# MarvinLvn/CPC2

Measured on AMD Instinct MI355X. Metric: audio-seconds/sec CPC training (1.28 s @16 kHz, 128 neg), higher is better.
Workload: dtype f32

## Files before the change

cpc2_amd/csrc/gru.hip:

```cpp
#include "common.h"
#include "coop.h"
#include "recurrent.h"

#include <algorithm>
#include <cstdlib>

namespace cpc {

__global__ void gru_pack_fwd_kernel(const float *w, float4 *wf, int H)
{
    const int total = 3 * H * (H / 4);
    for (int idx = blockIdx.x * blockDim.x + threadIdx.x; idx < total; idx += gridDim.x * blockDim.x) {
        const int j = idx % H;
        const int g = (idx / H) % 3;
        const int k4 = idx / (3 * H);
        const float *src = w + (long)(g * H + j) * H + 4 * k4;
        wf[idx] = make_float4(src[0], src[1], src[2], src[3]);
    }
}

__global__ void gru_pack_bwd_kernel(const float *w, float4 *wb, int H)
{
    const int total = (3 * H / 4) * H;
    for (int idx = blockIdx.x * blockDim.x + threadIdx.x; idx < total; idx += gridDim.x * blockDim.x) {
        const int j = idx % H;
        const int g4 = idx / H;
        wb[idx] = make_float4(w[(long)(4 * g4) * H + j], w[(long)(4 * g4 + 1) * H + j], w[(long)(4 * g4 + 2) * H + j],
                              w[(long)(4 * g4 + 3) * H + j]);
    }
}

__device__ __forceinline__ float sigmoidf_(float x) { return 1.f / (1.f + expf(-x)); }

struct GruArgs {
    const float *gi;
    const float4 *wpack;
    const float *whh;
    const float *bhh;
    const float *h0;
    float *out;
    float *hall;
    float *gates;
    float *hn;
    float *hlast;
    int N, T, H;
    int hp, kq;
    const float *dout;
    float *dgi;
    float *dgh;
};

__global__ void gru_fwd_kernel(GruArgs a)
{
    extern __shared__ __attribute__((aligned(16))) float smem[];
    const int H = a.H, T = a.T, hp = a.hp, kq = a.kq;
    float *hs = smem;
    float *red = smem + ((H + 3) / 4) * 4;
    const int j = threadIdx.x % hp, q = threadIdx.x / hp;
    const bool act = j < H;
    const int n = blockIdx.x;
    const int k4_per = (H / 4 + kq - 1) / kq;
    const int k4_lo = q * k4_per, k4_hi = min(H / 4, k4_lo + k4_per);

    float hprev = 0.f;
    float bh[3] = {0.f, 0.f, 0.f};
    if (act && q == 0) {
        hprev = a.h0 != nullptr ? a.h0[(long)n * H + j] : 0.f;
        hs[j] = hprev;
        a.hall[((long)n * (T + 1)) * H + j] = hprev;
        bh[0] = a.bhh[j]; bh[1] = a.bhh[H + j]; bh[2] = a.bhh[2 * H + j];
    }
    __syncthreads();

    for (int t = 0; t < T; ++t) {
        float acc0 = 0.f, acc1 = 0.f, acc2 = 0.f;
        if (act) {
            const float4 *wp = a.wpack + j;
#pragma unroll 4
            for (int k4 = k4_lo; k4 < k4_hi; ++k4) {
                const float4 wr = wp[(long)(k4 * 3 + 0) * H];
                const float4 wz = wp[(long)(k4 * 3 + 1) * H];
                const float4 wn = wp[(long)(k4 * 3 + 2) * H];
                const float4 h4 = reinterpret_cast<const float4 *>(hs)[k4];
                acc0 = fmaf(wr.x, h4.x, fmaf(wr.y, h4.y, fmaf(wr.z, h4.z, fmaf(wr.w, h4.w, acc0))));
                acc1 = fmaf(wz.x, h4.x, fmaf(wz.y, h4.y, fmaf(wz.z, h4.z, fmaf(wz.w, h4.w, acc1))));
                acc2 = fmaf(wn.x, h4.x, fmaf(wn.y, h4.y, fmaf(wn.z, h4.z, fmaf(wn.w, h4.w, acc2))));
            }
            red[(q * 3 + 0) * hp + j] = acc0;
            red[(q * 3 + 1) * hp + j] = acc1;
            red[(q * 3 + 2) * hp + j] = acc2;
        }
        __syncthreads();
        if (act && q == 0) {
            float g0 = bh[0], g1 = bh[1], g2 = bh[2];
            for (int qq = 0; qq < kq; ++qq) {
                g0 += red[(qq * 3 + 0) * hp + j];
                g1 += red[(qq * 3 + 1) * hp + j];
                g2 += red[(qq * 3 + 2) * hp + j];
            }
            const long row = (long)n * T + t;
            const float *g = a.gi + row * 3 * H;
            const float r = sigmoidf_(g[j] + g0);
            const float z = sigmoidf_(g[H + j] + g1);
            const float c = tanhf(g[2 * H + j] + r * g2);
            const float hv = (1.f - z) * c + z * hprev;
            float *gs = a.gates + row * 3 * H;
            gs[j] = r; gs[H + j] = z; gs[2 * H + j] = c;
            a.hn[row * H + j] = g2;
            a.out[row * H + j] = hv;
            a.hall[((long)n * (T + 1) + t + 1) * H + j] = hv;
            hs[j] = hv;
            hprev = hv;
        }
        __syncthreads();
    }
    if (act && q == 0 && a.hlast != nullptr) a.hlast[(long)n * H + j] = hprev;
}

__global__ void gru_bwd_kernel(GruArgs a)
{
    extern __shared__ __attribute__((aligned(16))) float smem[];
    const int H = a.H, T = a.T, hp = a.hp, kq = a.kq;
    float *dg = smem;
    float *red = smem + 3 * H;
    const int j = threadIdx.x % hp, q = threadIdx.x / hp;
    const bool act = j < H;
    const int n = blockIdx.x;
    const int g4_total = 3 * H / 4;
    const int g4_per = (g4_total + kq - 1) / kq;
    const int g4_lo = q * g4_per, g4_hi = min(g4_total, g4_lo + g4_per);

    float carry = 0.f;
    if (act && q == 0) {
        float *zr = a.dgh + ((long)n * (T + 1) + T) * 3 * H;
        zr[j] = 0.f; zr[H + j] = 0.f; zr[2 * H + j] = 0.f;
    }
    for (int t = T - 1; t >= 0; --t) {
        float keep = 0.f;
        if (act && q == 0) {
            const long row = (long)n * T + t;
            const float dh = a.dout[row * H + j] + carry;
            const float *gs = a.gates + row * 3 * H;
            const float r = gs[j], z = gs[H + j], c = gs[2 * H + j];
            const float hnv = a.hn[row * H + j];
            const float hp_ = a.hall[((long)n * (T + 1) + t) * H + j];
            const float dc = dh * (1.f - z);
            const float dz = dh * (hp_ - c);
            const float dpn = dc * (1.f - c * c);
            const float dpr = dpn * hnv * r * (1.f - r);
            const float dpz = dz * z * (1.f - z);
            const float dhn = dpn * r;
            keep = dh * z;
            float *gi = a.dgi + row * 3 * H;
            gi[j] = dpr; gi[H + j] = dpz; gi[2 * H + j] = dpn;
            float *gh = a.dgh + ((long)n * (T + 1) + t) * 3 * H;
            gh[j] = dpr; gh[H + j] = dpz; gh[2 * H + j] = dhn;
            dg[j] = dpr; dg[H + j] = dpz; dg[2 * H + j] = dhn;
        }
        __syncthreads();
        if (act) {
            float acc = 0.f;
            const float4 *wp = a.wpack + j;
#pragma unroll 4
            for (int g4 = g4_lo; g4 < g4_hi; ++g4) {
                const float4 w4 = wp[(long)g4 * H];
                const float4 d4 = reinterpret_cast<const float4 *>(dg)[g4];
                acc = fmaf(w4.x, d4.x, fmaf(w4.y, d4.y, fmaf(w4.z, d4.z, fmaf(w4.w, d4.w, acc))));
            }
            red[q * hp + j] = acc;
        }
        __syncthreads();
        if (act && q == 0) {
            float sum = keep;
            for (int qq = 0; qq < kq; ++qq) sum += red[qq * hp + j];
            carry = sum;
        }
    }
}

struct GruCoopArgs {
    GruArgs g;
    gu64_t *comm;
    unsigned epoch0;
    int groups, xcd_map;
    int *err;
    int fault;
};

template <int H, int NB> __global__ __launch_bounds__(512) void gru_fwd_coop_kernel(GruCoopArgs ca)
{
    using C = CoopCfg<H>;
    constexpr int QS = C::QS, U = C::U, G = C::G;
    constexpr int KP = NB * H / 512 > 0 ? NB * H / 512 : 1;
    static_assert(NB <= QS, "one finishing lane per window");
    __shared__ __attribute__((aligned(16))) float hs[2][NB][C::LDH];
    const GruArgs &a = ca.g;
    const int T = a.T;
    int group, member;
    coop_who<G>(ca.groups, ca.xcd_map, group, member);
    const int tid = threadIdx.x;
    const int q = tid & (QS - 1), u = tid / QS;
    const int j = member * U + u;
    const int n0 = group * NB;

    f32x2 w[3][16];
#pragma unroll
    for (int g = 0; g < 3; ++g)
#pragma unroll
        for (int i4 = 0; i4 < 8; ++i4) {
            const float4 v = *reinterpret_cast<const float4 *>(a.whh + (long)(g * H + j) * H + q * 32 + 4 * i4);
            w[g][2 * i4] = pk_lo(v); w[g][2 * i4 + 1] = pk_hi(v);
        }
    const float bh0 = a.bhh[j], bh1 = a.bhh[H + j], bh2 = a.bhh[2 * H + j];

    for (int idx = tid; idx < NB * H; idx += 512) {
        const int s = idx / H, k = idx - s * H;
        const int n = n0 + s;
        const float v = (n < a.N && a.h0 != nullptr) ? a.h0[(long)n * H + k] : 0.f;
        hs[0][s][coop_pad(k)] = v;
        if (n < a.N && (k / U) == member) a.hall[((long)n * (T + 1)) * H + k] = v;
    }
    __syncthreads();

    const int ns = n0 + q;
    const bool mine = q < NB && ns < a.N;
    float gin0 = 0.f, gin1 = 0.f, gin2 = 0.f;
    if (mine) {
        const float *gp = a.gi + (long)ns * T * 3 * H;
        gin0 = gp[j]; gin1 = gp[H + j]; gin2 = gp[2 * H + j];
    }
    bool dead = false;
    for (int t = 0; t < T; ++t) {
        const int cur = t & 1, nxt = cur ^ 1;
        const float gi0 = gin0, gi1 = gin1, gi2 = gin2;
        if (mine && t + 1 < T) {
            const float *gp = a.gi + ((long)ns * T + t + 1) * 3 * H;
            gin0 = gp[j]; gin1 = gp[H + j]; gin2 = gp[2 * H + j];
        }
        float acc[NB][3];
#pragma unroll
        for (int s = 0; s < NB; ++s) {
            f32x2 a2[3] = {f32x2{0.f, 0.f}, f32x2{0.f, 0.f}, f32x2{0.f, 0.f}};
#pragma unroll
            for (int i4 = 0; i4 < 8; ++i4) {
                const float4 h4 = *reinterpret_cast<const float4 *>(&hs[cur][s][q * 36 + 4 * i4]);
#pragma unroll
                for (int g = 0; g < 3; ++g)
                    a2[g] = pk_fma(w[g][2 * i4 + 1], pk_hi(h4), pk_fma(w[g][2 * i4], pk_lo(h4), a2[g]));
            }
#pragma unroll
            for (int g = 0; g < 3; ++g) acc[s][g] = coop_group_sum<QS>(a2[g].x + a2[g].y);
        }
        if (q < NB) {
            float g0 = 0.f, g1 = 0.f, g2 = 0.f;
#pragma unroll
            for (int s = 0; s < NB; ++s)
                if (s == q) { g0 = acc[s][0]; g1 = acc[s][1]; g2 = acc[s][2]; }
            g0 += bh0; g1 += bh1; g2 += bh2;
            const float hp = hs[cur][q][coop_pad(j)];
            const float r = sigmoidf_(gi0 + g0);
            const float z = sigmoidf_(gi1 + g1);
            const float c = tanhf(gi2 + r * g2);
            float hv = (1.f - z) * c + z * hp;
            if (dead) hv = NAN;
            COOP_GLOBAL gu64_t *slot = (COOP_GLOBAL gu64_t *)(ca.comm + coop_fwd_slot<H, NB>(group, nxt, member, u, q));
            if (!(ca.fault && group == 0 && member == 0 && t == 1))
                __hip_atomic_store(slot, ((gu64_t)(ca.epoch0 + (unsigned)(t + 1)) << 32) | (gu64_t)__float_as_uint(mine ? hv : 0.f),
                                   __ATOMIC_RELAXED, __HIP_MEMORY_SCOPE_AGENT);
            if (mine) {
                const long row = (long)ns * T + t;
                float *gs = a.gates + row * 3 * H;
                gs[j] = r; gs[H + j] = z; gs[2 * H + j] = c;
                a.hn[row * H + j] = g2;
                a.out[row * H + j] = hv;
                a.hall[((long)ns * (T + 1) + t + 1) * H + j] = hv;
            }
        }
        if (t + 1 < T) {
            COOP_GLOBAL gu64_t *slot[KP];
#pragma unroll
            for (int i = 0; i < KP; ++i) {
                const int idx = tid + 512 * i;
                slot[i] = (COOP_GLOBAL gu64_t *)(ca.comm + ((long)group * 2 + nxt) * (NB * H) + idx);
            }
            gu64_t x[KP];
            unsigned spins = dead ? (1u << 22) : 0u;
            if (tid < NB * H) {
                for (;;) {
                    bool ready = true;
#pragma unroll
                    for (int i = 0; i < KP; ++i) x[i] = __hip_atomic_load(slot[i], __ATOMIC_RELAXED, __HIP_MEMORY_SCOPE_AGENT);
#pragma unroll
                    for (int i = 0; i < KP; ++i) ready = ready && (unsigned)(x[i] >> 32) == ca.epoch0 + (unsigned)(t + 1);
                    if (ready) break;
                    if (++spins > (1u << 22)) { dead = true; coop_report(ca.err, COOP_ERR_FWD_WAIT); break; }
                    __builtin_amdgcn_s_sleep(1);
                }
#pragma unroll
                for (int i = 0; i < KP; ++i) {
                    const int idx = tid + 512 * i;
                    int gw, gk;
                    coop_fwd_who<H, NB>(idx, gw, gk);
                    hs[nxt][gw][coop_pad(gk)] = dead ? NAN : __uint_as_float((unsigned)x[i]);
                }
            }
            coop_lds_barrier();
        }
    }
    if (a.hlast != nullptr && q < NB && n0 + q < a.N)
        a.hlast[(long)(n0 + q) * H + j] = a.hall[((long)(n0 + q) * (T + 1) + T) * H + j];
}

typedef float f32x4_t __attribute__((ext_vector_type(4)));
typedef __bf16 bf16x8_t __attribute__((ext_vector_type(8)));
struct MfmaFrag { unsigned d[4]; };

__device__ __forceinline__ unsigned short bf16_rne(float v) { return __builtin_bit_cast(unsigned short, (__bf16)v); }
__device__ __forceinline__ void split3(float v, unsigned short (&t)[3])
{
    t[0] = bf16_rne(v);
    v -= __uint_as_float((unsigned)t[0] << 16);
    t[1] = bf16_rne(v);
    v -= __uint_as_float((unsigned)t[1] << 16);
    t[2] = bf16_rne(v);
}

template <int H> struct MfmaCfg {
    using C = CoopCfg<H>;
    static constexpr int N3 = 3 * C::U;
    static constexpr int TILES = N3 / 16;
    static constexpr int KS = 24 / TILES;
    static constexpr int KPU = (H / 32) / KS;
    static constexpr int LDK = H + 8;
    static_assert(N3 % 16 == 0 && 24 % TILES == 0 && (H / 32) % KS == 0 && KPU == 4, "24 units of 4 K steps");
};

template <int H, int NB> __global__ __launch_bounds__(512) void gru_fwd_mfma_kernel(GruCoopArgs ca)
{
    using C = CoopCfg<H>;
    using M = MfmaCfg<H>;
    constexpr int QS = C::QS, U = C::U, G = C::G;
    constexpr int KP = NB * H / 512 > 0 ? NB * H / 512 : 1;
    constexpr int LDK = M::LDK;
    static_assert(NB <= 8 && NB <= QS, "eight windows fill half the rows of a 16-row tile");
    __shared__ __attribute__((aligned(16))) unsigned short hp[2][3][8][LDK];
    __shared__ __attribute__((aligned(16))) unsigned short zrow[LDK];
    __shared__ __attribute__((aligned(16))) float part[24][16][16];
    const GruArgs &a = ca.g;
    const int T = a.T;
    int group, member;
    coop_who<G>(ca.groups, ca.xcd_map, group, member);
    const int tid = threadIdx.x, lane = tid & 63;
    const int wave = __builtin_amdgcn_readfirstlane(tid >> 6);
    const int q = tid & (QS - 1), u = tid / QS;
    const int j = member * U + u;
    const int n0 = group * NB;

    MfmaFrag bw[3][4][3];
    const int kpart = wave % M::KS, tile0 = 3 * (wave / M::KS);
#pragma unroll
    for (int i = 0; i < 3; ++i) {
        const int tile = tile0 + i;
        const int col = tile * 16 + (lane & 15);
        const long row = (long)((col / U) * H + member * U + (col % U)) * H;
#pragma unroll
        for (int ks = 0; ks < 4; ++ks) {
            const int k = (kpart * 4 + ks) * 32 + 8 * (lane >> 4);
            const float4 v0 = *reinterpret_cast<const float4 *>(a.whh + row + k);
            const float4 v1 = *reinterpret_cast<const float4 *>(a.whh + row + k + 4);
            const float v[8] = {v0.x, v0.y, v0.z, v0.w, v1.x, v1.y, v1.z, v1.w};
            unsigned short t[8][3];
#pragma unroll
            for (int e = 0; e < 8; ++e) split3(v[e], t[e]);
#pragma unroll
            for (int pl = 0; pl < 3; ++pl)
#pragma unroll
                for (int d = 0; d < 4; ++d) bw[i][ks][pl].d[d] = (unsigned)t[2 * d][pl] | ((unsigned)t[2 * d + 1][pl] << 16);
        }
    }
    const float bh0 = a.bhh[j], bh1 = a.bhh[H + j], bh2 = a.bhh[2 * H + j];

    for (int idx = tid; idx < 8 * H; idx += 512) {
        const int s = idx / H, k = idx - s * H;
        const int n = n0 + s;
        const float v = (s < NB && n < a.N && a.h0 != nullptr) ? a.h0[(long)n * H + k] : 0.f;
        unsigned short t[3];
        split3(v, t);
#pragma unroll
        for (int pl = 0; pl < 3; ++pl) { hp[0][pl][s][k] = t[pl]; hp[1][pl][s][k] = 0; }
        if (s < NB && n < a.N && (k / U) == member) a.hall[((long)n * (T + 1)) * H + k] = v;
    }
    for (int k = tid; k < LDK; k += 512) zrow[k] = 0;
    __syncthreads();

    const int ns = n0 + q;
    const bool mine = q < NB && ns < a.N;
    float hprev = (mine && a.h0 != nullptr) ? a.h0[(long)ns * H + j] : 0.f;
    float gin0 = 0.f, gin1 = 0.f, gin2 = 0.f;
    if (mine) {
        const float *gp = a.gi + (long)ns * T * 3 * H;
        gin0 = gp[j]; gin1 = gp[H + j]; gin2 = gp[2 * H + j];
    }
    const int arow = lane & 15, akg = lane >> 4;
    const unsigned aoff0 = (unsigned)(((0 * 8 + (arow & 7)) * LDK + 8 * akg) * 2);
    const unsigned aoff1 = (unsigned)(((1 * 8 + (arow & 7)) * LDK + 8 * akg) * 2);
    const unsigned aoff2 = (unsigned)(((2 * 8 + (arow & 7)) * LDK + 8 * akg) * 2);
    const bool upper = arow >= 8;
    int ptile[3], pcol[3];
#pragma unroll
    for (int g = 0; g < 3; ++g) { ptile[g] = (g * U + u) / 16; pcol[g] = (g * U + u) % 16; }
    bool dead = false;
    for (int t = 0; t < T; ++t) {
        const int cur = t & 1, nxt = cur ^ 1;
        const float gi0 = gin0, gi1 = gin1, gi2 = gin2;
        if (mine && t + 1 < T) {
            const float *gp = a.gi + ((long)ns * T + t + 1) * 3 * H;
            gin0 = gp[j]; gin1 = gp[H + j]; gin2 = gp[2 * H + j];
        }
        const char *planes = reinterpret_cast<const char *>(&hp[cur][0][0][0]);
        const char *pa1 = planes + (upper ? aoff1 : aoff0);
        const char *pa2 = planes + (upper ? aoff2 : aoff0);
        const char *pa3 = upper ? reinterpret_cast<const char *>(zrow) + 16 * akg : planes + aoff2;
        f32x4_t acc[3];
#pragma unroll
        for (int i = 0; i < 3; ++i) acc[i] = f32x4_t{0.f, 0.f, 0.f, 0.f};
#pragma unroll
        for (int ks = 0; ks < 4; ++ks) {
            const int kb = (kpart * 4 + ks) * 64;
            const bf16x8_t a1 = *reinterpret_cast<const bf16x8_t *>(pa1 + kb);
            const bf16x8_t a2 = *reinterpret_cast<const bf16x8_t *>(pa2 + kb);
            const bf16x8_t a3 = *reinterpret_cast<const bf16x8_t *>(pa3 + (upper ? 0 : kb));
#pragma unroll
            for (int i = 0; i < 3; ++i) {
                acc[i] = __builtin_amdgcn_mfma_f32_16x16x32_bf16(a1, __builtin_bit_cast(bf16x8_t, bw[i][ks][0]), acc[i], 0, 0, 0);
                acc[i] = __builtin_amdgcn_mfma_f32_16x16x32_bf16(a1, __builtin_bit_cast(bf16x8_t, bw[i][ks][1]), acc[i], 0, 0, 0);
                acc[i] = __builtin_amdgcn_mfma_f32_16x16x32_bf16(a2, __builtin_bit_cast(bf16x8_t, bw[i][ks][2]), acc[i], 0, 0, 0);
                acc[i] = __builtin_amdgcn_mfma_f32_16x16x32_bf16(a3, __builtin_bit_cast(bf16x8_t, bw[i][ks][0]), acc[i], 0, 0, 0);
            }
        }
#pragma unroll
        for (int i = 0; i < 3; ++i)
            *reinterpret_cast<f32x4_t *>(&part[(tile0 + i) * M::KS + kpart][lane & 15][4 * (lane >> 4)]) = acc[i];
        coop_lds_barrier();
        if (q < NB) {
            float gs[3];
#pragma unroll
            for (int g = 0; g < 3; ++g) {
                float v = 0.f;
#pragma unroll
                for (int p = 0; p < M::KS; ++p) {
                    v += part[ptile[g] * M::KS + p][pcol[g]][q];
                    v += part[ptile[g] * M::KS + p][pcol[g]][q + 8];
                }
                gs[g] = v;
            }
            const float g0 = gs[0] + bh0, g1 = gs[1] + bh1, g2 = gs[2] + bh2;
            const float r = sigmoidf_(gi0 + g0);
            const float z = sigmoidf_(gi1 + g1);
            const float c = tanhf(gi2 + r * g2);
            float hv = (1.f - z) * c + z * hprev;
            if (dead) hv = NAN;
            hprev = hv;
            COOP_GLOBAL gu64_t *slot = (COOP_GLOBAL gu64_t *)(ca.comm + coop_fwd_slot<H, NB>(group, nxt, member, u, q));
            if (!(ca.fault && group == 0 && member == 0 && t == 1))
                __hip_atomic_store(slot, ((gu64_t)(ca.epoch0 + (unsigned)(t + 1)) << 32) | (gu64_t)__float_as_uint(mine ? hv : 0.f),
                                   __ATOMIC_RELAXED, __HIP_MEMORY_SCOPE_AGENT);
            if (mine) {
                const long row = (long)ns * T + t;
                float *gsv = a.gates + row * 3 * H;
                gsv[j] = r; gsv[H + j] = z; gsv[2 * H + j] = c;
                a.hn[row * H + j] = g2;
                a.out[row * H + j] = hv;
                a.hall[((long)ns * (T + 1) + t + 1) * H + j] = hv;
            }
        }
        if (t + 1 < T) {
            COOP_GLOBAL gu64_t *slot[KP];
#pragma unroll
            for (int i = 0; i < KP; ++i)
                slot[i] = (COOP_GLOBAL gu64_t *)(ca.comm + ((long)group * 2 + nxt) * (NB * H) + tid + 512 * i);
            gu64_t x[KP];
            unsigned spins = dead ? (1u << 22) : 0u;
            if (tid < NB * H) {
                for (;;) {
                    bool ready = true;
#pragma unroll
                    for (int i = 0; i < KP; ++i) x[i] = __hip_atomic_load(slot[i], __ATOMIC_RELAXED, __HIP_MEMORY_SCOPE_AGENT);
#pragma unroll
                    for (int i = 0; i < KP; ++i) ready = ready && (unsigned)(x[i] >> 32) == ca.epoch0 + (unsigned)(t + 1);
                    if (ready) break;
                    if (++spins > (1u << 22)) { dead = true; coop_report(ca.err, COOP_ERR_FWD_WAIT); break; }
                    __builtin_amdgcn_s_sleep(1);
                }
#pragma unroll
                for (int i = 0; i < KP; ++i) {
                    int gw, gk;
                    coop_fwd_who<H, NB>(tid + 512 * i, gw, gk);
                    unsigned short tt[3];
                    split3(dead ? NAN : __uint_as_float((unsigned)x[i]), tt);
#pragma unroll
                    for (int pl = 0; pl < 3; ++pl) hp[nxt][pl][gw][gk] = tt[pl];
                }
            }
            coop_lds_barrier();
        }
    }
    if (a.hlast != nullptr && q < NB && n0 + q < a.N) a.hlast[(long)(n0 + q) * H + j] = hprev;
}

template <int H, int NB> __global__ __launch_bounds__(512) void gru_bwd_coop_kernel(GruCoopArgs ca)
{
    using C = CoopCfg<H>;
    constexpr int U = C::U, G = C::G, HALVES = C::HALVES;
    static_assert(3 * U / HALVES == 96, "96 weights per thread");
    static_assert(NB * U <= 512, "one elementwise thread per (window, unit)");
    __shared__ __attribute__((aligned(16))) float dgs[NB][3 * U];
    __shared__ float part[HALVES][NB][H];
    const GruArgs &a = ca.g;
    const int T = a.T;
    int group, member;
    coop_who<G>(ca.groups, ca.xcd_map, group, member);
    const int tid = threadIdx.x;
    const int jc = tid & (H - 1), half = tid / H;
    const int n0 = group * NB;

    f32x2 w[48];
#pragma unroll
    for (int i = 0; i < 96; ++i) {
        const int lr = half * 96 + i;
        w[i / 2][i % 2] = a.whh[(long)((lr / U) * H + member * U + (lr % U)) * H + jc];
    }
    const int es = tid / U, eu = tid - es * U;
    const int ej = member * U + eu;
    const int en = n0 + es;
    const bool ew = tid < NB * U;
    const bool emine = ew && en < a.N;
    float carry = 0.f;
    if (emine) {
        float *zr = a.dgh + ((long)en * (T + 1) + T) * 3 * H;
        zr[ej] = 0.f; zr[H + ej] = 0.f; zr[2 * H + ej] = 0.f;
    }
    float p_dout = 0.f, p_r = 0.f, p_z = 0.f, p_c = 0.f, p_hn = 0.f, p_hp = 0.f;
    auto request = [&](int t) {
        const long row = (long)en * T + t;
        const float *gs = a.gates + row * 3 * H;
        p_dout = a.dout[row * H + ej];
        p_r = gs[ej]; p_z = gs[H + ej]; p_c = gs[2 * H + ej];
        p_hn = a.hn[row * H + ej];
        p_hp = a.hall[((long)en * (T + 1) + t) * H + ej];
    };
    if (emine) request(T - 1);
    coop_weights_ready(w);
    bool dead = false;
    for (int t = T - 1; t >= 0; --t) {
        const int par = t & 1;
        const unsigned epoch = ca.epoch0 + (unsigned)(T - t);
        float keep = 0.f;
        if (ew) {
            float dpr = 0.f, dpz = 0.f, dhn = 0.f;
            if (emine) {
                const long row = (long)en * T + t;
                const float dh = p_dout + carry;
                const float r = p_r, z = p_z, c = p_c;
                const float hnv = p_hn;
                const float hp_ = p_hp;
                const float dc = dh * (1.f - z);
                const float dz = dh * (hp_ - c);
                const float dpn = dc * (1.f - c * c);
                dpr = dpn * hnv * r * (1.f - r);
                dpz = dz * z * (1.f - z);
                dhn = dpn * r;
                keep = dh * z;
                float *gi = a.dgi + row * 3 * H;
                gi[ej] = dpr; gi[H + ej] = dpz; gi[2 * H + ej] = dpn;
                float *gh = a.dgh + ((long)en * (T + 1) + t) * 3 * H;
                gh[ej] = dpr; gh[H + ej] = dpz; gh[2 * H + ej] = dhn;
            }
            dgs[es][eu] = dpr; dgs[es][U + eu] = dpz; dgs[es][2 * U + eu] = dhn;
            if (emine && t > 0) request(t - 1);
        }
        coop_lds_barrier();
        f32x2 acc[NB];
#pragma unroll
        for (int s = 0; s < NB; ++s) acc[s] = f32x2{0.f, 0.f};
#pragma unroll
        for (int i4 = 0; i4 < 24; ++i4) {
#pragma unroll
            for (int s = 0; s < NB; ++s) {
                const float4 d4 = *reinterpret_cast<const float4 *>(&dgs[s][half * 96 + 4 * i4]);
                acc[s] = pk_fma(w[2 * i4 + 1], pk_hi(d4), pk_fma(w[2 * i4], pk_lo(d4), acc[s]));
            }
        }
#pragma unroll
        for (int s = 0; s < NB; ++s) part[half][s][jc] = acc[s].x + acc[s].y;
        coop_lds_barrier();
        auto column = [&](int s, int k) {
            float v = part[0][s][k];
#pragma unroll
            for (int hh = 1; hh < HALVES; ++hh) v += part[hh][s][k];
            return v;
        };
        if (t > 0) {
            for (int idx = tid; idx < NB * H; idx += 512) {
                const int s = idx / H, k = idx - s * H;
                if (k / U == member) continue;
                const float v = column(s, k);
                COOP_GLOBAL gu64_t *slot =
                    (COOP_GLOBAL gu64_t *)(ca.comm + ((((long)group * 2 + par) * G + member) * NB + s) * H + k);
                __hip_atomic_store(slot, ((gu64_t)epoch << 32) | (gu64_t)__float_as_uint(dead ? NAN : v), __ATOMIC_RELAXED,
                                   __HIP_MEMORY_SCOPE_AGENT);
            }
            if (ew) {
                float sum = keep + column(es, ej);
                COOP_GLOBAL gu64_t *slot[G - 1];
#pragma unroll
                for (int d = 1; d < G; ++d) {
                    const int src = (member + d) & (G - 1);
                    slot[d - 1] = (COOP_GLOBAL gu64_t *)(ca.comm + ((((long)group * 2 + par) * G + src) * NB + es) * H + ej);
                }
                gu64_t x[G - 1];
                unsigned spins = dead ? (1u << 22) : 0u;
                for (;;) {
                    bool ready = true;
#pragma unroll
                    for (int d = 0; d < G - 1; ++d) x[d] = __hip_atomic_load(slot[d], __ATOMIC_RELAXED, __HIP_MEMORY_SCOPE_AGENT);
#pragma unroll
                    for (int d = 0; d < G - 1; ++d) ready = ready && (unsigned)(x[d] >> 32) == epoch;
                    if (ready) break;
                    if (++spins > (1u << 22)) { dead = true; coop_report(ca.err, COOP_ERR_BWD_WAIT); break; }
                    __builtin_amdgcn_s_sleep(1);
                }
#pragma unroll
                for (int d = 0; d < G - 1; ++d) sum += __uint_as_float((unsigned)x[d]);
                carry = dead ? NAN : sum;
            }
        }
    }
}

template <int H, int NB> __global__ __launch_bounds__(512) void gru_bwd_mfma_kernel(GruCoopArgs ca)
{
    using C = CoopCfg<H>;
    constexpr int U = C::U, G = C::G;
    constexpr int K3 = 3 * U, LDK = K3 + 8;
    constexpr int TW = H / 16 / 8;
    static_assert(K3 % 32 == 0 && TW * 8 * 16 == H && TW * (K3 / 32) == 12, "twelve (tile, K step) operands per wave, all of K each");
    static_assert(NB <= 8 && NB * U <= 512, "one elementwise thread per (window, unit)");
    __shared__ __attribute__((aligned(16))) unsigned short dgp[3][8][LDK];
    __shared__ __attribute__((aligned(16))) unsigned short zrow[LDK];
    __shared__ float part[2][8][H];
    const GruArgs &a = ca.g;
    const int T = a.T;
    int group, member;
    coop_who<G>(ca.groups, ca.xcd_map, group, member);
    const int tid = threadIdx.x, lane = tid & 63;
    const int wave = __builtin_amdgcn_readfirstlane(tid >> 6);
    const int n0 = group * NB;

    MfmaFrag bw[TW][K3 / 32][3];
#pragma unroll
    for (int i = 0; i < TW; ++i) {
        const int jcol = (wave * TW + i) * 16 + (lane & 15);
#pragma unroll
        for (int ks = 0; ks < K3 / 32; ++ks) {
            unsigned short t[8][3];
#pragma unroll
            for (int e = 0; e < 8; ++e) {
                const int lr = ks * 32 + 8 * (lane >> 4) + e;
                split3(a.whh[(long)((lr / U) * H + member * U + (lr % U)) * H + jcol], t[e]);
            }
#pragma unroll
            for (int pl = 0; pl < 3; ++pl)
#pragma unroll
                for (int d = 0; d < 4; ++d) bw[i][ks][pl].d[d] = (unsigned)t[2 * d][pl] | ((unsigned)t[2 * d + 1][pl] << 16);
        }
    }
    for (int idx = tid; idx < 3 * 8 * LDK; idx += 512) (&dgp[0][0][0])[idx] = 0;
    for (int kk = tid; kk < LDK; kk += 512) zrow[kk] = 0;
    __syncthreads();
    const int arow = lane & 15, akg = lane >> 4;
    const bool upper = arow >= 8;
    const char *const planes = reinterpret_cast<const char *>(&dgp[0][0][0]);
    const char *const pa1 = planes + (((upper ? 1 : 0) * 8 + (arow & 7)) * LDK + 8 * akg) * 2;
    const char *const pa2 = planes + (((upper ? 2 : 0) * 8 + (arow & 7)) * LDK + 8 * akg) * 2;
    const char *const pa3 = upper ? reinterpret_cast<const char *>(zrow) + 16 * akg : planes + ((2 * 8 + arow) * LDK + 8 * akg) * 2;
    const int es = tid / U, eu = tid - es * U;
    const int ej = member * U + eu;
    const int en = n0 + es;
    const bool ew = tid < NB * U;
    const bool emine = ew && en < a.N;
    float carry = 0.f;
    if (emine) {
        float *zr = a.dgh + ((long)en * (T + 1) + T) * 3 * H;
        zr[ej] = 0.f; zr[H + ej] = 0.f; zr[2 * H + ej] = 0.f;
    }
    float p_dout = 0.f, p_r = 0.f, p_z = 0.f, p_c = 0.f, p_hn = 0.f, p_hp = 0.f;
    auto request = [&](int t) {
        const long row = (long)en * T + t;
        const float *gs = a.gates + row * 3 * H;
        p_dout = a.dout[row * H + ej];
        p_r = gs[ej]; p_z = gs[H + ej]; p_c = gs[2 * H + ej];
        p_hn = a.hn[row * H + ej];
        p_hp = a.hall[((long)en * (T + 1) + t) * H + ej];
    };
    if (emine) request(T - 1);
    bool dead = false;
    for (int t = T - 1; t >= 0; --t) {
        const int par = t & 1;
        const unsigned epoch = ca.epoch0 + (unsigned)(T - t);
        float keep = 0.f;
        if (ew) {
            float dpr = 0.f, dpz = 0.f, dhn = 0.f;
            if (emine) {
                const long row = (long)en * T + t;
                const float dh = p_dout + carry;
                const float r = p_r, z = p_z, c = p_c;
                const float hnv = p_hn;
                const float hp_ = p_hp;
                const float dc = dh * (1.f - z);
                const float dz = dh * (hp_ - c);
                const float dpn = dc * (1.f - c * c);
                dpr = dpn * hnv * r * (1.f - r);
                dpz = dz * z * (1.f - z);
                dhn = dpn * r;
                keep = dh * z;
                float *gi = a.dgi + row * 3 * H;
                gi[ej] = dpr; gi[H + ej] = dpz; gi[2 * H + ej] = dpn;
                float *gh = a.dgh + ((long)en * (T + 1) + t) * 3 * H;
                gh[ej] = dpr; gh[H + ej] = dpz; gh[2 * H + ej] = dhn;
            }
            {
                unsigned short t0[3], t1[3], t2[3];
                split3(dpr, t0); split3(dpz, t1); split3(dhn, t2);
#pragma unroll
                for (int pl = 0; pl < 3; ++pl) { dgp[pl][es][eu] = t0[pl]; dgp[pl][es][U + eu] = t1[pl]; dgp[pl][es][2 * U + eu] = t2[pl]; }
            }
            if (emine && t > 0) request(t - 1);
        }
        coop_lds_barrier();
        {
            f32x4_t acc[TW];
#pragma unroll
            for (int i = 0; i < TW; ++i) acc[i] = f32x4_t{0.f, 0.f, 0.f, 0.f};
#pragma unroll
            for (int ks = 0; ks < K3 / 32; ++ks) {
                const bf16x8_t a1 = *reinterpret_cast<const bf16x8_t *>(pa1 + ks * 64);
                const bf16x8_t a2 = *reinterpret_cast<const bf16x8_t *>(pa2 + ks * 64);
                const bf16x8_t a3 = *reinterpret_cast<const bf16x8_t *>(pa3 + (upper ? 0 : ks * 64));
#pragma unroll
                for (int i = 0; i < TW; ++i) {
                    acc[i] = __builtin_amdgcn_mfma_f32_16x16x32_bf16(a1, __builtin_bit_cast(bf16x8_t, bw[i][ks][0]), acc[i], 0, 0, 0);
                    acc[i] = __builtin_amdgcn_mfma_f32_16x16x32_bf16(a1, __builtin_bit_cast(bf16x8_t, bw[i][ks][1]), acc[i], 0, 0, 0);
                    acc[i] = __builtin_amdgcn_mfma_f32_16x16x32_bf16(a2, __builtin_bit_cast(bf16x8_t, bw[i][ks][2]), acc[i], 0, 0, 0);
                    acc[i] = __builtin_amdgcn_mfma_f32_16x16x32_bf16(a3, __builtin_bit_cast(bf16x8_t, bw[i][ks][0]), acc[i], 0, 0, 0);
                }
            }
#pragma unroll
            for (int i = 0; i < TW; ++i) {
                const int col = (wave * TW + i) * 16 + (lane & 15);
#pragma unroll
                for (int e = 0; e < 4; ++e) part[lane >> 5][4 * ((lane >> 4) & 1) + e][col] = acc[i][e];
            }
        }
        coop_lds_barrier();
        auto column = [&](int s, int k) { return part[0][s][k] + part[1][s][k]; };
        if (t > 0) {
            for (int idx = tid; idx < NB * H; idx += 512) {
                const int s = idx / H, k = idx - s * H;
                if (k / U == member) continue;
                const float v = column(s, k);
                COOP_GLOBAL gu64_t *slot =
                    (COOP_GLOBAL gu64_t *)(ca.comm + ((((long)group * 2 + par) * G + member) * NB + s) * H + k);
                __hip_atomic_store(slot, ((gu64_t)epoch << 32) | (gu64_t)__float_as_uint(dead ? NAN : v), __ATOMIC_RELAXED,
                                   __HIP_MEMORY_SCOPE_AGENT);
            }
            if (ew) {
                float sum = keep + column(es, ej);
                COOP_GLOBAL gu64_t *slot[G - 1];
#pragma unroll
                for (int d = 1; d < G; ++d) {
                    const int src = (member + d) & (G - 1);
                    slot[d - 1] = (COOP_GLOBAL gu64_t *)(ca.comm + ((((long)group * 2 + par) * G + src) * NB + es) * H + ej);
                }
                gu64_t x[G - 1];
                unsigned spins = dead ? (1u << 22) : 0u;
                for (;;) {
                    bool ready = true;
#pragma unroll
                    for (int d = 0; d < G - 1; ++d) x[d] = __hip_atomic_load(slot[d], __ATOMIC_RELAXED, __HIP_MEMORY_SCOPE_AGENT);
#pragma unroll
                    for (int d = 0; d < G - 1; ++d) ready = ready && (unsigned)(x[d] >> 32) == epoch;
                    if (ready) break;
                    if (++spins > (1u << 22)) { dead = true; coop_report(ca.err, COOP_ERR_BWD_WAIT); break; }
                    __builtin_amdgcn_s_sleep(1);
                }
#pragma unroll
                for (int d = 0; d < G - 1; ++d) sum += __uint_as_float((unsigned)x[d]);
                carry = dead ? NAN : sum;
            }
        }
    }
}


static bool mfma_wanted(int H, int nb, bool backward)
{
    static const bool off = getenv("CPC_GRU_NO_MFMA") != nullptr, all = getenv("CPC_GRU_MFMA_ALL") != nullptr;
    if (off) return false;
    return all || (H == 512 && nb == 8) || (backward && H == 256 && nb >= 2);
}

struct GruCell {
    static constexpr int G = 3;
    static constexpr const char *name = "gru", *kernel_names[2] = {"gru_fwd_kernel", "gru_bwd_kernel"},
                                *pack_names[2] = {"gru_pack_fwd_kernel", "gru_pack_bwd_kernel"};
    using Args = GruArgs;
    using CoopArgs = GruCoopArgs;
    using CoopKernel = void (*)(GruCoopArgs);
    static constexpr auto fwd_kernel = gru_fwd_kernel, bwd_kernel = gru_bwd_kernel;

    static void take_saved(RecLayout &g, Carver &sv, int l)
    {
        g.gates[l] = sv.take<float>((size_t)g.N * g.T * 3 * g.H);
        g.extra[l] = sv.take<float>((size_t)g.N * g.T * g.H);
        g.hall[l] = sv.take<float>((size_t)g.N * (g.T + 1) * g.H);
    }
    static void cell_args(GruArgs &a, float *hn, const float *, float *) { a.hn = hn; }
    static void pack(bool backward, const float *w_hh, float4 *wpack, int H, hipStream_t st)
    {
        hipLaunchKernelGGL((backward ? gru_pack_bwd_kernel : gru_pack_fwd_kernel), dim3(256), dim3(256), 0, st, w_hh, wpack, H);
    }
    template <auto Plain, auto Mfma> static CoopKernel pick(bool mfma)
    {
        if (!coop_kernel_fits<Plain>()) return nullptr;
        return mfma && coop_kernel_fits<Mfma>() ? Mfma : Plain;
    }
    static CoopKernel coop_kernel(bool backward, int H, int nb)
    {
        return coop_dispatch(H, nb, [&](auto h, auto n) -> CoopKernel {
            constexpr int HH = decltype(h)::value, NB = decltype(n)::value;
            if (backward) return pick<gru_bwd_coop_kernel<HH, NB>, gru_bwd_mfma_kernel<HH, NB>>(mfma_wanted(HH, NB, true));
            return pick<gru_fwd_coop_kernel<HH, NB>, gru_fwd_mfma_kernel<HH, NB>>(mfma_wanted(HH, NB, false));
        });
    }
};

}

using cpc::GruCell;

extern "C" size_t cpc_gru_saved_bytes(int n, int t, int dim_in, int hidden, int layers)
{
    return cpc::rec_bytes<GruCell>(&cpc::RecLayout::saved_bytes, n, t, dim_in, hidden, layers);
}

extern "C" size_t cpc_gru_scratch_bytes(int n, int t, int dim_in, int hidden, int layers)
{
    return cpc::rec_bytes<GruCell>(&cpc::RecLayout::scratch_bytes, n, t, dim_in, hidden, layers);
}

extern "C" int cpc_gru_forward(const float *x, const float *const *params, const float *h0, float *out, float *h_last,
                               void *saved, void *scratch, int n, int t, int dim_in, int hidden, int layers, cpc_stream_t stream)
{
    CPC_TRY(cpc::coop_error_take("cpc_gru_forward"));
    return cpc::rec_forward<GruCell>(x, params, h0, nullptr, out, h_last, nullptr, saved, scratch, n, t, dim_in, hidden, layers,
                                     static_cast<hipStream_t>(stream));
}

extern "C" int cpc_gru_backward(const float *x, const float *const *params, const float *dout, void *saved, void *scratch,
                                float *dx, float *const *grads, int n, int t, int dim_in, int hidden, int layers, int deferred,
                                cpc_stream_t stream)
{
    cpc::coop_count_backward_call();
    CPC_TRY(cpc::coop_error_take("cpc_gru_backward"));
    return cpc::rec_backward<GruCell>(x, params, dout, saved, scratch, dx, grads, n, t, dim_in, hidden, layers,
                                      static_cast<hipStream_t>(stream), deferred != 0);
}
```

cpc2_amd/csrc/ldsdma.h:

```cpp
#pragma once
#include <hip/hip_runtime.h>

namespace cpc {

typedef unsigned frag_t __attribute__((ext_vector_type(4)));

__device__ __forceinline__ void glds16(unsigned lds_dst, unsigned voff, const void *sbase)
{
    unsigned keep;
    asm volatile("s_mov_b32 %0, m0\n\t"
                 "s_mov_b32 m0, %1\n\t"
                 "s_nop 0\n\t"
                 "global_load_lds_dwordx4 %2, %3\n\t"
                 "s_mov_b32 m0, %0"
                 : "=&s"(keep)
                 : "s"(lds_dst), "v"(voff), "s"(sbase)
                 : "memory");
}
__device__ __forceinline__ void glds16_addr(unsigned lds_dst, const void *lane_src)
{
    unsigned keep;
    asm volatile("s_mov_b32 %0, m0\n\t"
                 "s_mov_b32 m0, %1\n\t"
                 "s_nop 0\n\t"
                 "global_load_lds_dwordx4 %2, off\n\t"
                 "s_mov_b32 m0, %0"
                 : "=&s"(keep)
                 : "s"(lds_dst), "v"(lane_src)
                 : "memory");
}

#define CPC_GLDS_FIRST(MOD) "s_mov_b32 %0, m0\n\ts_sub_u32 m0, %1, %11\n\ts_nop 0\n\tglobal_load_lds_dwordx4 %2, %10 offset:%11" MOD "\n\t"
#define CPC_GLDS_NEXT(N, MOD) "s_add_u32 m0, m0, %12\n\ts_nop 0\n\tglobal_load_lds_dwordx4 %" #N ", %10 offset:%11" MOD "\n\t"
#define CPC_GLDS_BODY8(MOD)                                                                                                     \
    CPC_GLDS_FIRST(MOD) CPC_GLDS_NEXT(3, MOD) CPC_GLDS_NEXT(4, MOD) CPC_GLDS_NEXT(5, MOD) CPC_GLDS_NEXT(6, MOD) CPC_GLDS_NEXT(7, MOD)   \
    CPC_GLDS_NEXT(8, MOD) CPC_GLDS_NEXT(9, MOD)
#define CPC_GLDS_OPS                                                                                                              \
    : "=&s"(keep)                                                                                                                \
    : "s"(lds_dst), "v"(vo[0]), "v"(vo[1]), "v"(vo[2]), "v"(vo[3]), "v"(vo[4]), "v"(vo[5]), "v"(vo[6]), "v"(vo[7]), "s"(sbase), "n"(GOFF), \
      "n"(PSTEP)                                                                                                                 \
    : "memory", "scc"
template <int PSTEP, int GOFF, bool NT = false>
__device__ __forceinline__ void glds16x8(unsigned lds_dst, const unsigned (&vo)[8], const void *sbase)
{
    unsigned keep;
    if constexpr (NT) asm volatile(CPC_GLDS_BODY8(" nt") "s_mov_b32 m0, %0" CPC_GLDS_OPS);
    else asm volatile(CPC_GLDS_BODY8("") "s_mov_b32 m0, %0" CPC_GLDS_OPS);
}
#undef CPC_GLDS_OPS

typedef unsigned u32x2_t __attribute__((ext_vector_type(2)));
template <int D0, int D1> __device__ __forceinline__ u32x2_t lds_read2(unsigned addr)
{
    u32x2_t v;
    asm volatile("ds_read2_b32 %0, %1 offset0:%2 offset1:%3" : "=v"(v) : "v"(addr), "n"(D0), "n"(D1) : "memory");
    return v;
}

template <int OFF> __device__ __forceinline__ frag_t lds_read16(unsigned addr)
{
    frag_t v;
    asm volatile("ds_read_b128 %0, %1 offset:%2" : "=v"(v) : "v"(addr), "n"(OFF) : "memory");
    return v;
}

__device__ __forceinline__ unsigned lds_addr(const void *p) { return (unsigned)(unsigned long long)p; }

}
```

Before: 17380.

## Offload GRU coop per-step global loads/stores to a dedicated memory wave with LDS ring

When the cooperative GRU forward/backward kernels have a spare wave (NB*H or NB*U below 512 threads), one wave is made a memory wave. It prefetches the per-step inputs (gi, or dout/gates/hn/hall) several steps ahead into an LDS ring using global_load_lds. It also drains the per-step outputs from an LDS staging buffer to global memory, so the compute waves on the serial recurrence critical path avoid global latency. This adds LDS usage, hand-tuned vmcnt waits and extra complexity in the step-by-step synchronization.

```diff
diff --git a/cpc2_amd/csrc/gru.hip b/cpc2_amd/csrc/gru.hip
--- a/cpc2_amd/csrc/gru.hip
+++ b/cpc2_amd/csrc/gru.hip
@@ -1,5 +1,6 @@
 #include "common.h"
 #include "coop.h"
+#include "ldsdma.h"
 #include "recurrent.h"
 
 #include <algorithm>
@@ -178,6 +179,8 @@
     }
 }
 
+constexpr int COOP_RING = 4;
+
 struct GruCoopArgs {
     GruArgs g;
     gu64_t *comm;
@@ -193,12 +196,18 @@
     constexpr int QS = C::QS, U = C::U, G = C::G;
     constexpr int KP = NB * H / 512 > 0 ? NB * H / 512 : 1;
     static_assert(NB <= QS, "one finishing lane per window");
+    constexpr bool MW = NB * H < 512;
+    constexpr int MWAVE = NB * H / 64, ME = MW ? NB * U : 1;
+    static_assert(!MW || NB * U == 64, "the memory wave's operations are counted for one full wave of (window, unit) pairs");
     __shared__ __attribute__((aligned(16))) float hs[2][NB][C::LDH];
+    __shared__ __attribute__((aligned(16))) float gring[MW ? COOP_RING : 1][3][ME];
+    __shared__ float stage[2][5][ME];
     const GruArgs &a = ca.g;
     const int T = a.T;
     int group, member;
     coop_who<G>(ca.groups, ca.xcd_map, group, member);
     const int tid = threadIdx.x;
+    const bool memwave = MW && __builtin_amdgcn_readfirstlane(tid >> 6) == MWAVE;
     const int q = tid & (QS - 1), u = tid / QS;
     const int j = member * U + u;
     const int n0 = group * NB;
@@ -211,7 +220,11 @@
             const float4 v = *reinterpret_cast<const float4 *>(a.whh + (long)(g * H + j) * H + q * 32 + 4 * i4);
             w[g][2 * i4] = pk_lo(v); w[g][2 * i4 + 1] = pk_hi(v);
         }
-    const float bh0 = a.bhh[j], bh1 = a.bhh[H + j], bh2 = a.bhh[2 * H + j];
+    float bh0 = a.bhh[j], bh1 = a.bhh[H + j], bh2 = a.bhh[2 * H + j];
+    if constexpr (MW) {
+        coop_weights_ready(w[0]); coop_weights_ready(w[1]); coop_weights_ready(w[2]);
+        asm volatile("" : "+v"(bh0), "+v"(bh1), "+v"(bh2));
+    }
 
     for (int idx = tid; idx < NB * H; idx += 512) {
         const int s = idx / H, k = idx - s * H;
@@ -220,22 +233,58 @@
         hs[0][s][coop_pad(k)] = v;
         if (n < a.N && (k / U) == member) a.hall[((long)n * (T + 1)) * H + k] = v;
     }
+    const int me = tid & 63, mn = n0 + me / U, mj = member * U + me % U;
+    const bool mreal = mn < a.N;
+    const float *const mgi = a.gi + (long)min(mn, a.N - 1) * T * 3 * H + mj;
+    auto prefetch = [&](int step) {
+        const float *gp = mgi + (long)min(step, T - 1) * 3 * H;
+        const unsigned dst = lds_addr(&gring[step & (COOP_RING - 1)][0][0]);
+#pragma unroll
+        for (int g = 0; g < 3; ++g) glds4_addr(dst + g * ME * 4, gp + g * H);
+    };
+    auto write_out = [&](int step) {
+        if (mreal) {
+            const float(&sg)[5][ME] = stage[step & 1];
+            const long row = (long)mn * T + step;
+            float *gs = a.gates + row * 3 * H;
+            gs[mj] = sg[0][me]; gs[H + mj] = sg[1][me]; gs[2 * H + mj] = sg[2][me];
+            a.hn[row * H + mj] = sg[3][me];
+            a.out[row * H + mj] = sg[4][me];
+            a.hall[((long)mn * (T + 1) + step + 1) * H + mj] = sg[4][me];
+        }
+    };
+    if constexpr (MW) {
+        if (memwave) {
+            for (int k = 0; k < COOP_RING - 1; ++k) prefetch(k);
+            asm volatile("s_waitcnt vmcnt(0)" ::: "memory");
+        }
+    }
     __syncthreads();
 
     const int ns = n0 + q;
     const bool mine = q < NB && ns < a.N;
     float gin0 = 0.f, gin1 = 0.f, gin2 = 0.f;
-    if (mine) {
-        const float *gp = a.gi + (long)ns * T * 3 * H;
-        gin0 = gp[j]; gin1 = gp[H + j]; gin2 = gp[2 * H + j];
-    }
+    if constexpr (!MW) {
+        if (mine) {
+            const float *gp = a.gi + (long)ns * T * 3 * H;
+            gin0 = gp[j]; gin1 = gp[H + j]; gin2 = gp[2 * H + j];
+        }
+    }
+    float hfin = 0.f;
     bool dead = false;
     for (int t = 0; t < T; ++t) {
         const int cur = t & 1, nxt = cur ^ 1;
-        const float gi0 = gin0, gi1 = gin1, gi2 = gin2;
-        if (mine && t + 1 < T) {
-            const float *gp = a.gi + ((long)ns * T + t + 1) * 3 * H;
-            gin0 = gp[j]; gin1 = gp[H + j]; gin2 = gp[2 * H + j];
+        float gi0 = gin0, gi1 = gin1, gi2 = gin2;
+        if constexpr (MW) {
+            if (q < NB) {
+                const float(&rg)[3][ME] = gring[t & (COOP_RING - 1)];
+                gi0 = rg[0][q * U + u]; gi1 = rg[1][q * U + u]; gi2 = rg[2][q * U + u];
+            }
+        } else {
+            if (mine && t + 1 < T) {
+                const float *gp = a.gi + ((long)ns * T + t + 1) * 3 * H;
+                gin0 = gp[j]; gin1 = gp[H + j]; gin2 = gp[2 * H + j];
+            }
         }
         float acc[NB][3];
 #pragma unroll
@@ -267,7 +316,12 @@
             if (!(ca.fault && group == 0 && member == 0 && t == 1))
                 __hip_atomic_store(slot, ((gu64_t)(ca.epoch0 + (unsigned)(t + 1)) << 32) | (gu64_t)__float_as_uint(mine ? hv : 0.f),
                                    __ATOMIC_RELAXED, __HIP_MEMORY_SCOPE_AGENT);
-            if (mine) {
+            if constexpr (MW) {
+                float(&sg)[5][ME] = stage[t & 1];
+                const int e = q * U + u;
+                sg[0][e] = r; sg[1][e] = z; sg[2][e] = c; sg[3][e] = g2; sg[4][e] = hv;
+                hfin = hv;
+            } else if (mine) {
                 const long row = (long)ns * T + t;
                 float *gs = a.gates + row * 3 * H;
                 gs[j] = r; gs[H + j] = z; gs[2 * H + j] = c;
@@ -276,6 +330,14 @@
                 a.hall[((long)ns * (T + 1) + t + 1) * H + j] = hv;
             }
         }
+        if constexpr (MW) {
+            if (memwave) {
+                if (t > 0) write_out(t - 1);
+                prefetch(t + COOP_RING - 1);
+                if (ca.fault) asm volatile("s_waitcnt vmcnt(0)" ::: "memory");
+                else asm volatile("s_waitcnt vmcnt(20)" ::: "memory");
+            }
+        }
         if (t + 1 < T) {
             COOP_GLOBAL gu64_t *slot[KP];
 #pragma unroll
@@ -307,8 +369,17 @@
             coop_lds_barrier();
         }
     }
-    if (a.hlast != nullptr && q < NB && n0 + q < a.N)
-        a.hlast[(long)(n0 + q) * H + j] = a.hall[((long)(n0 + q) * (T + 1) + T) * H + j];
+    if constexpr (MW) {
+        __syncthreads();
+        if (memwave) {
+            write_out(T - 1);
+            asm volatile("s_waitcnt vmcnt(0)" ::: "memory");
+        }
+        if (a.hlast != nullptr && mine) a.hlast[(long)ns * H + j] = hfin;
+    } else {
+        if (a.hlast != nullptr && q < NB && n0 + q < a.N)
+            a.hlast[(long)(n0 + q) * H + j] = a.hall[((long)(n0 + q) * (T + 1) + T) * H + j];
+    }
 }
 
 typedef float f32x4_t __attribute__((ext_vector_type(4)));
@@ -514,13 +585,18 @@
     constexpr int U = C::U, G = C::G, HALVES = C::HALVES;
     static_assert(3 * U / HALVES == 96, "96 weights per thread");
     static_assert(NB * U <= 512, "one elementwise thread per (window, unit)");
+    constexpr bool MW = NB * U < 512;
+    constexpr int MWAVE = (NB * U + 63) / 64, ME = MW ? NB * U : 1, MI = (ME + 63) / 64;
     __shared__ __attribute__((aligned(16))) float dgs[NB][3 * U];
     __shared__ float part[HALVES][NB][H];
+    __shared__ __attribute__((aligned(16))) float ring[MW ? COOP_RING : 1][6][MI * 64];
+    __shared__ float stage[2][4][ME];
     const GruArgs &a = ca.g;
     const int T = a.T;
     int group, member;
     coop_who<G>(ca.groups, ca.xcd_map, group, member);
     const int tid = threadIdx.x;
+    const bool memwave = MW && __builtin_amdgcn_readfirstlane(tid >> 6) == MWAVE;
     const int jc = tid & (H - 1), half = tid / H;
     const int n0 = group * NB;
 
@@ -536,10 +612,6 @@
     const bool ew = tid < NB * U;
     const bool emine = ew && en < a.N;
     float carry = 0.f;
-    if (emine) {
-        float *zr = a.dgh + ((long)en * (T + 1) + T) * 3 * H;
-        zr[ej] = 0.f; zr[H + ej] = 0.f; zr[2 * H + ej] = 0.f;
-    }
     float p_dout = 0.f, p_r = 0.f, p_z = 0.f, p_c = 0.f, p_hn = 0.f, p_hp = 0.f;
     auto request = [&](int t) {
         const long row = (long)en * T + t;
@@ -549,7 +621,57 @@
         p_hn = a.hn[row * H + ej];
         p_hp = a.hall[((long)en * (T + 1) + t) * H + ej];
     };
-    if (emine) request(T - 1);
+    const int mlane = tid & 63;
+    auto prefetch = [&](int step) {
+        const int tt = max(step, 0);
+#pragma unroll
+        for (int i = 0; i < MI; ++i) {
+            const int e = mlane + 64 * i, mn = n0 + e / U, mj = member * U + e % U;
+            if (e < ME && mn < a.N) {
+                const long row = (long)mn * T + tt;
+                const unsigned dst = lds_addr(&ring[step & (COOP_RING - 1)][0][64 * i]);
+                glds4_addr(dst, a.dout + row * H + mj);
+#pragma unroll
+                for (int g = 0; g < 3; ++g) glds4_addr(dst + (1 + g) * MI * 256, a.gates + row * 3 * H + g * H + mj);
+                glds4_addr(dst + 4 * MI * 256, a.hn + row * H + mj);
+                glds4_addr(dst + 5 * MI * 256, a.hall + ((long)mn * (T + 1) + tt) * H + mj);
+            }
+        }
+    };
+    auto write_out = [&](int step) {
+        const float(&sg)[4][ME] = stage[step & 1];
+#pragma unroll
+        for (int i = 0; i < MI; ++i) {
+            const int e = mlane + 64 * i, mn = n0 + e / U, mj = member * U + e % U;
+            if (e < ME && mn < a.N) {
+                float *gi = a.dgi + ((long)mn * T + step) * 3 * H;
+                gi[mj] = sg[0][e]; gi[H + mj] = sg[1][e]; gi[2 * H + mj] = sg[2][e];
+                float *gh = a.dgh + ((long)mn * (T + 1) + step) * 3 * H;
+                gh[mj] = sg[0][e]; gh[H + mj] = sg[1][e]; gh[2 * H + mj] = sg[3][e];
+            }
+        }
+    };
+    if constexpr (MW) {
+        if (memwave) {
+#pragma unroll
+            for (int i = 0; i < MI; ++i) {
+                const int e = mlane + 64 * i, mn = n0 + e / U, mj = member * U + e % U;
+                if (e < ME && mn < a.N) {
+                    float *zr = a.dgh + ((long)mn * (T + 1) + T) * 3 * H;
+                    zr[mj] = 0.f; zr[H + mj] = 0.f; zr[2 * H + mj] = 0.f;
+                }
+            }
+            for (int k = 1; k <= COOP_RING; ++k) prefetch(T - k);
+            asm volatile("s_waitcnt vmcnt(0)" ::: "memory");
+        }
+        __syncthreads();
+    } else {
+        if (emine) {
+            float *zr = a.dgh + ((long)en * (T + 1) + T) * 3 * H;
+            zr[ej] = 0.f; zr[H + ej] = 0.f; zr[2 * H + ej] = 0.f;
+        }
+        if (emine) request(T - 1);
+    }
     coop_weights_ready(w);
     bool dead = false;
     for (int t = T - 1; t >= 0; --t) {
@@ -559,7 +681,10 @@
         if (ew) {
             float dpr = 0.f, dpz = 0.f, dhn = 0.f;
             if (emine) {
-                const long row = (long)en * T + t;
+                if constexpr (MW) {
+                    const float(&rg)[6][MI * 64] = ring[t & (COOP_RING - 1)];
+                    p_dout = rg[0][tid]; p_r = rg[1][tid]; p_z = rg[2][tid]; p_c = rg[3][tid]; p_hn = rg[4][tid]; p_hp = rg[5][tid];
+                }
                 const float dh = p_dout + carry;
                 const float r = p_r, z = p_z, c = p_c;
                 const float hnv = p_hn;
@@ -571,13 +696,20 @@
                 dpz = dz * z * (1.f - z);
                 dhn = dpn * r;
                 keep = dh * z;
-                float *gi = a.dgi + row * 3 * H;
-                gi[ej] = dpr; gi[H + ej] = dpz; gi[2 * H + ej] = dpn;
-                float *gh = a.dgh + ((long)en * (T + 1) + t) * 3 * H;
-                gh[ej] = dpr; gh[H + ej] = dpz; gh[2 * H + ej] = dhn;
+                if constexpr (MW) {
+                    float(&sg)[4][ME] = stage[par];
+                    sg[0][tid] = dpr; sg[1][tid] = dpz; sg[2][tid] = dpn; sg[3][tid] = dhn;
+                } else {
+                    const long row = (long)en * T + t;
+                    float *gi = a.dgi + row * 3 * H;
+                    gi[ej] = dpr; gi[H + ej] = dpz; gi[2 * H + ej] = dpn;
+                    float *gh = a.dgh + ((long)en * (T + 1) + t) * 3 * H;
+                    gh[ej] = dpr; gh[H + ej] = dpz; gh[2 * H + ej] = dhn;
+                }
             }
             dgs[es][eu] = dpr; dgs[es][U + eu] = dpz; dgs[es][2 * U + eu] = dhn;
-            if (emine && t > 0) request(t - 1);
+            if constexpr (!MW)
+                if (emine && t > 0) request(t - 1);
         }
         coop_lds_barrier();
         f32x2 acc[NB];
@@ -635,7 +767,16 @@
                 carry = dead ? NAN : sum;
             }
         }
-    }
+        if constexpr (MW) {
+            if (memwave) {
+                write_out(t);
+                prefetch(t - COOP_RING);
+                asm volatile("s_waitcnt vmcnt(24)" ::: "memory");
+            }
+        }
+    }
+    if constexpr (MW)
+        if (memwave) asm volatile("s_waitcnt vmcnt(0)" ::: "memory");
 }
 
 template <int H, int NB> __global__ __launch_bounds__(512) void gru_bwd_mfma_kernel(GruCoopArgs ca)
diff --git a/cpc2_amd/csrc/ldsdma.h b/cpc2_amd/csrc/ldsdma.h
--- a/cpc2_amd/csrc/ldsdma.h
+++ b/cpc2_amd/csrc/ldsdma.h
@@ -24,6 +24,19 @@
                  "s_mov_b32 m0, %1\n\t"
                  "s_nop 0\n\t"
                  "global_load_lds_dwordx4 %2, off\n\t"
+                 "s_mov_b32 m0, %0"
+                 : "=&s"(keep)
+                 : "s"(lds_dst), "v"(lane_src)
+                 : "memory");
+}
+
+__device__ __forceinline__ void glds4_addr(unsigned lds_dst, const void *lane_src)
+{
+    unsigned keep;
+    asm volatile("s_mov_b32 %0, m0\n\t"
+                 "s_mov_b32 m0, %1\n\t"
+                 "s_nop 0\n\t"
+                 "global_load_lds_dword %2, off\n\t"
                  "s_mov_b32 m0, %0"
                  : "=&s"(keep)
                  : "s"(lds_dst), "v"(lane_src)
```

After: 17590 (median of 6 runs). 1.2% higher.
